# lxd99/TPNet

Hardware: AMD Instinct MI355X
Metric: temporal edges/sec (proj-update + pairwise readout) (higher is better)
Workload: dtype f32; 1 GPU; C2: Wikipedia-shape d=128 B=1000, L=3, synthetic S(8227,1000,E,span) stream of 2399000 edges, decoder-level unit (2 readouts + update per edge); batch=1000, dim=128, num_layer=3, nodes=9228, parallelism=single GPU

## Files before the change

### tpnet_amd/csrc/wplan_dense.hip

```cpp
#include "wplan_dense.hpp"

namespace tpnet {

static constexpr int64_t DENSE_SHARD_MAX_BATCH = 8192;
bool wplan_dense_eligible(int64_t N, int d, int L, int64_t batch) {
    static const int off = TPNET_DEV_INT(NO_PLAN_DENSE, 0);
    if (off || batch < 1 || batch > DENSE_SHARD_MAX_BATCH || N > (int64_t)DENSE_MAX_CHUNKS * 256) return false;
    return (int64_t)N * 12 <= batch * (int64_t)L * d * 4;
}

size_t wplan_dense_bytes(int64_t Ec, int64_t batch, int64_t N, int d, int L) {
    if (!wplan_dense_eligible(N, d, L, batch)) return 0;
    return measured([&](Arena& a) { DView v; dense_layout(a, v, Ec, batch, N); });
}

struct DArgs {
    const int64_t* src;
    const int64_t* dst;
    const int64_t* neg;
    const double* t;
    const double* t_prev;
    const NodeMeta* meta;
    uint32_t* err;
    int64_t Ec, Bfull, N, nb, nw;
    double now_time, lambda;
    int32_t node_bits, L, nwhich , nchunks;
    int64_t own;
    uint32_t* status;
};

__device__ __forceinline__ void dense_place(const WPlan& p, const WTmp& q, const DView& D, const DArgs& a,
                                            const uint32_t* __restrict__ lstart, const uint32_t* __restrict__ cbase,
                                            const double* tl, int64_t x) {
    const BatchDesc* __restrict__ desc = p.base.desc;
    const int KW = p.K;
    const int64_t b = x / (2 * a.Bfull);
    const int64_t e0b = b * a.Bfull;
    const int64_t neb = (a.Ec - e0b < a.Bfull) ? (a.Ec - e0b) : a.Bfull;
    const uint32_t node = q.bkey[x];
    const int32_t partner = q.bpart[x];
    const float coef = q.bcoef[x];
    const uint32_t ri = q.bri[x];
    const uint32_t fl = q.bflags[x] & WT_STRUCT_MASK;
    const uint32_t val = q.bval[x];
    const uint2 mo = D.m[b * D.Ns + node];
    const uint2 mp = D.m[b * D.Ns + (uint32_t)partner];
    const uint2 wsl_own = (fl & WREF_RUN_HEAD) ? D.wsl[(b / KW) * D.Ns + node] : make_uint2(0u, 0u);
    const uint32_t bo = D.base[node] + cbase[node / (uint32_t)DCH];
    const uint32_t bp = D.base[(uint32_t)partner] + cbase[(uint32_t)partner / (uint32_t)DCH];
    const uint4 o0 = reinterpret_cast<const uint4*>(a.meta + node)[0], o1 = reinterpret_cast<const uint4*>(a.meta + node)[1];
    const uint4 p0 = reinterpret_cast<const uint4*>(a.meta + partner)[0], p1 = reinterpret_cast<const uint4*>(a.meta + partner)[1];
    const double Tb = desc[b].t_last, Tnow = desc[b].now;
    const DVRef own = dense_version(desc, tl, mo, bo, o0, o1);
    const DVRef pr = dense_version(desc, tl, mp, bp, p0, p1);
    const uint32_t f = bo + mo.x + ri;
    uint32_t out = fl | pr.ref;
    float dec = 1.0f;
    if (fl & WREF_RUN_HEAD) {
        const int64_t w = b / KW;
        const uint32_t prevb = mo.y >> 16;
        const bool chain_head = mo.x == 0u || (int64_t)prevb < w * KW;
        if (chain_head) {
            float g_first = 1.0f;
            if (own.ref & WREF_TABLE) g_first = decay3_f32(a.lambda, Tb - own.t_src);
            else dec = decay3_f32(a.lambda, Tb - own.t_src);
            const uint32_t cnt = wsl_own.x;
            const int c = wchain_class(cnt, p.heavy_thr);
            const uint32_t pair = (uint32_t)w * 8u + (uint32_t)c;
            const uint32_t chunk = node / (uint32_t)DCH;
            const uint32_t at = lstart[pair] + D.cpre[(size_t)chunk * (size_t)(a.nw * 8) + pair] + D.crank[w * D.Ns + node];
            uint4* rec = reinterpret_cast<uint4*>(p.chains + at);
            rec[0] = make_uint4(f, cnt, node, own.ref);
            rec[1] = make_uint4(__float_as_uint(g_first), 0u, 0u, 0u);
        } else {
            dec = decay3_f32(a.lambda, Tb - own.t_src);
        }
    }
    if ((fl & WREF_RUN_TAIL) && D.lastb[node] == (uint32_t)b) out |= WREF_LAST_RUN;
    wrec_store(p.rec, f, partner, coef, out, decay3_f32(a.lambda, Tb - pr.t_src), dec, (int32_t)node, (uint32_t)b);
    if (a.nwhich >= 2) {
        const bool side = val >= (uint32_t)neb;
        const int64_t e = e0b + (side ? (int64_t)val - neb : (int64_t)val);
        p.e_ref[(side ? a.Ec : 0) + e] = own.ref;
        p.e_g[(side ? a.Ec : 0) + e] = decay3_f32(a.lambda, Tnow - own.t_src);
    }
}

__device__ __forceinline__ void dense_neg(const WPlan& p, const DView& D, const DArgs& a, const uint32_t* __restrict__ basef,
                                          int64_t e) {
    const BatchDesc* __restrict__ desc = p.base.desc;
    int64_t node = a.neg[e];
    if ((uint64_t)node >= (uint64_t)a.N) node = 0;
    const int64_t b = e / a.Bfull;
    const uint2 m = D.m[b * D.Ns + node];
    const uint32_t bs = basef[node];
    const uint4 m0 = reinterpret_cast<const uint4*>(a.meta + node)[0], m1 = reinterpret_cast<const uint4*>(a.meta + node)[1];
    const DVRef r = dense_version(desc, nullptr, m, bs, m0, m1);
    p.e_ref[2 * a.Ec + e] = r.ref;
    p.e_g[2 * a.Ec + e] = decay3_f32(a.lambda, desc[b].now - r.t_src);
}

__device__ __forceinline__ void dense_neg_c(const WPlan& p, const DView& D, const DArgs& a, const uint32_t* __restrict__ cbase,
                                            const double* tl, int64_t e, int which = 2) {
    const BatchDesc* __restrict__ desc = p.base.desc;
    int64_t node = which == 2 ? a.neg[e] : a.dst[e];
    if ((uint64_t)node >= (uint64_t)a.N) node = 0;
    if (which == 1 && node < a.own) return;
    const int64_t b = e / a.Bfull;
    const uint2 m = D.m[b * D.Ns + node];
    const uint32_t bs = D.base[node] + cbase[(uint32_t)node / (uint32_t)DCH];
    const uint4 m0 = reinterpret_cast<const uint4*>(a.meta + node)[0], m1 = reinterpret_cast<const uint4*>(a.meta + node)[1];
    const DVRef r = dense_version(desc, tl, m, bs, m0, m1);
    p.e_ref[(int64_t)which * a.Ec + e] = r.ref;
    p.e_g[(int64_t)which * a.Ec + e] = decay3_f32(a.lambda, desc[b].now - r.t_src);
}

template <int BS, int IPT>
__global__ __launch_bounds__(BS) void k_dense_sort(WPlan p, WTmp q, DView D, DArgs a) {
    __shared__ WSortShared<BS, IPT> sh;
    const int64_t bb = blockIdx.x;
    wsort_batch<BS, IPT, true>(sh, q, p.base.desc, a.src, a.dst, a.t, a.Ec, (int32_t)a.Bfull, a.N, a.node_bits, a.now_time,
                               a.t_prev, a.lambda, a.L, a.err, p.K, bb, D.len + bb * D.Ns);
}


static constexpr int DENSE_GROUP_MAX_N = 12288;
template <int BS, int IPT, int NT>
__global__ __launch_bounds__(BS) void k_dense_group(WPlan p, WTmp q, DView D, DArgs a) {
    constexpr int NC = BS * IPT;
    constexpr int SPT = NT / BS;
    static_assert(SPT * BS == NT && SPT % 4 == 0, "k_dense_group: table size");
    constexpr int NW = BS / 64;
    constexpr int BMW = NC / 32;
    constexpr uint32_t SMALL = 16;
    static_assert(NC <= 2048 && BMW <= 64, "k_dense_group: j fits 11 bits, a hub's bitmap one word per lane");
    const int64_t bb = blockIdx.x;
    const BatchSpan sp = batch_span(bb, a.src, a.dst, a.t, a.Ec, a.Bfull);
    const int64_t e0 = sp.e0;
    const int32_t B = sp.B;
    const int64_t g0 = 2 * e0;
    uint16_t* __restrict__ lenrow = D.len + bb * D.Ns;
    __shared__ __attribute__((aligned(16))) uint32_t tab[NT];
    __shared__ uint16_t mem[NC];
    __shared__ uint32_t sorted[NC];
    __shared__ uint32_t bm[NW][BMW];
    __shared__ uint32_t e_src[NC / 2], e_dst[NC / 2];
    __shared__ float e_w[NC / 2];
    __shared__ uint32_t n_big, wsum[NW];
    __shared__ uint32_t big[NC / SMALL];
    const int tid = threadIdx.x;
    const int nc = 2 * B;
    const auto burst = edges_load<BS, IPT / 2>(sp);
    const double t_now = batch_clock(bb, e0, a.t, a.t_prev, a.now_time);
    if (tid == 0) n_big = 0;
#pragma unroll
    for (int k = 0; k < SPT / 4; ++k) reinterpret_cast<uint4*>(tab)[k * BS + tid] = make_uint4(0u, 0u, 0u, 0u);
    edges_stage<BS>(burst, B, a.N, a.lambda, a.err, e_src, e_dst, e_w);
    __syncthreads();
    uint32_t key[IPT], arr[IPT];
#pragma unroll
    for (int k = 0; k < IPT; ++k) {
        const int j = k * BS + tid;
        key[k] = 0;
        arr[k] = 0;
        if (j < nc) {
            key[k] = contrib_target(j, B, e_src, e_dst);
            arr[k] = atomicAdd(&tab[key[k]], 1u);
        }
    }
    __syncthreads();
    uint32_t c[SPT], tsum = 0;
#pragma unroll
    for (int k = 0; k < SPT / 4; ++k) {
        const uint4 v = reinterpret_cast<const uint4*>(tab)[tid * (SPT / 4) + k];
        c[4 * k] = v.x; c[4 * k + 1] = v.y; c[4 * k + 2] = v.z; c[4 * k + 3] = v.w;
        tsum += v.x + v.y + v.z + v.w;
    }
#pragma unroll
    for (int k = 0; k < SPT; ++k) {
        const int64_t n = (int64_t)tid * SPT + k;
        if (n < a.N) lenrow[n] = (uint16_t)c[k];
    }
    uint32_t total;
    uint32_t base = block_excl_scan<BS, false>(tsum, wsum, total);
    if (tsum) {
#pragma unroll
        for (int k = 0; k < SPT; ++k) {
            tab[tid * SPT + k] = (base << 16) | c[k];
            if (c[k] > SMALL) big[atomicAdd(&n_big, 1u)] = (uint32_t)(tid * SPT + k);
            base += c[k];
        }
    }
    __syncthreads();
#pragma unroll
    for (int k = 0; k < IPT; ++k) {
        const int j = k * BS + tid;
        if (j < nc) mem[(tab[key[k]] >> 16) + arr[k]] = (uint16_t)j;
    }
    __syncthreads();
    rank_groups<BS, IPT, SMALL>(tab, key, nc, mem, big, n_big, bm, [&](uint32_t j, uint32_t gb, uint32_t rank, uint32_t cnt) {
        sorted[gb + rank] = j | (rank << 11) | ((cnt - 1u) << 22);
    });
    __syncthreads();
#pragma unroll
    for (int k = 0; k < IPT; ++k) {
        const int pos = k * BS + tid;
        if (pos < nc) {
            const uint32_t v = sorted[pos];
            const uint32_t j = v & 0x7FFu, ri = (v >> 11) & 0x7FFu, cnt = (v >> 22) + 1u;
            int32_t partner;
            float w;
            contrib_partner_weight((int)j, B, e_src, e_dst, e_w, partner, w);
            q.bkey[g0 + pos] = contrib_target((int)j, B, e_src, e_dst);
            q.bpart[g0 + pos] = partner;
            q.bcoef[g0 + pos] = w;
            q.bval[g0 + pos] = j;
            q.binv[g0 + j] = (uint32_t)(g0 + pos);
            q.bri[g0 + pos] = ri;
            q.bflags[g0 + pos] = wref_run_flags(ri, ri + 1u == cnt);
        }
    }
    if (tid == 0) batch_desc_store(p.base.desc, bb, sp, t_now, burst.t_last, 0u, 0u, false, a.lambda, a.L);
}

template <int BS, int IPT>
__global__ __launch_bounds__(BS) void k_dense_sort_shard(WPlan p, WTmp q, DView D, DArgs a) {
    using Sort = rocprim::block_radix_sort<uint32_t, BS, IPT, uint32_t>;
    constexpr int NC = BS * IPT;
    constexpr int CMAX = 16;
    __shared__ union U {
        typename Sort::storage_type sort;
        struct { uint32_t key[NC]; uint32_t ustart[NC]; } s;
        struct { uint32_t ckey[NC]; uint32_t cval[NC]; } c;
    } u;
    __shared__ uint32_t wsum[BS / 64];
    constexpr int HBITS = 2048;
    __shared__ uint32_t hbits[HBITS];
    static_assert(sizeof(U) + sizeof(uint32_t) * HBITS <= 62 * 1024, "k_dense_sort_shard: LDS budget");
    const int64_t bb = blockIdx.x;
    const int tid = threadIdx.x;
    const BatchSpan sp = batch_span(bb, a.src, a.dst, a.t, a.Ec, a.Bfull);
    const int64_t e0 = sp.e0;
    const int32_t B = sp.B;
    const int64_t* __restrict__ src = sp.src;
    const int64_t* __restrict__ dst = sp.dst;
    const double* __restrict__ t = sp.t;
    const int64_t g0 = 2 * e0;
    uint16_t* __restrict__ lenrow = D.len + bb * D.Ns;
    for (int i = tid; i < HBITS; i += BS) hbits[i] = 0u;
    const bool hfit = a.N - a.own <= (int64_t)HBITS * 32;
    for (int64_t n = tid; n < (hfit ? a.own : a.N); n += BS) lenrow[n] = 0;
    __syncthreads();
    const double t_last = t[B - 1];
    const int nall = 2 * B;
    const int C = (nall + BS - 1) / BS;
    uint32_t rk[CMAX];
    uint32_t kept = 0;
#pragma unroll
    for (int k = 0; k < CMAX; ++k) {
        rk[k] = 0xFFFFFFFFu;
        const int j = tid * C + k;
        if (k < C && j < nall) {
            const bool side = j >= B;
            const int e = side ? j - B : j;
            const int64_t sv = src[e], dv = dst[e];
            const bool ok = (uint64_t)sv < (uint64_t)a.N && (uint64_t)dv < (uint64_t)a.N;
            if (!ok) {
                if (!side) atomicAdd(a.err, 1u);
            } else {
                const int64_t tg = side ? dv : sv;
                if (tg < a.own) { rk[k] = (uint32_t)tg; ++kept; }
                else if (hfit) atomicOr(&hbits[(tg - a.own) >> 5], 1u << ((tg - a.own) & 31));
                else lenrow[tg] = 1;
            }
        }
    }
    uint32_t total;
    uint32_t off = block_excl_scan<BS>(kept, wsum, total);
    if (hfit)
        for (int64_t n = a.own + tid; n < a.N; n += BS) lenrow[n] = (uint16_t)((hbits[(n - a.own) >> 5] >> ((n - a.own) & 31)) & 1u);
    if (total > (uint32_t)NC) {
        if (tid == 0 && a.status) atomicAdd(a.status, 1u);
        total = NC;
    }
#pragma unroll
    for (int k = 0; k < CMAX; ++k) {
        if (rk[k] != 0xFFFFFFFFu) {
            if (off < (uint32_t)NC) { u.c.ckey[off] = rk[k]; u.c.cval[off] = (uint32_t)(tid * C + k); }
            ++off;
        }
    }
    __syncthreads();
    const int nc = (int)total;
    uint32_t keys[IPT], vals[IPT];
    const uint32_t pad_key = 1u << a.node_bits;
#pragma unroll
    for (int k = 0; k < IPT; ++k) {
        const int j = tid * IPT + k;
        keys[k] = j < nc ? u.c.ckey[j] : pad_key;
        vals[k] = j < nc ? u.c.cval[j] : 0u;
    }
    __syncthreads();
    Sort().sort(keys, vals, u.sort, 0u, (unsigned)(a.node_bits + 1));
    __syncthreads();
#pragma unroll
    for (int k = 0; k < IPT; ++k) u.s.key[tid * IPT + k] = keys[k];
    __syncthreads();
    uint32_t hcount = 0;
    bool hd[IPT];
#pragma unroll
    for (int k = 0; k < IPT; ++k) {
        const int j = tid * IPT + k;
        hd[k] = j < nc && (j == 0 || u.s.key[j - 1] != keys[k]);
        hcount += hd[k] ? 1u : 0u;
        if (j < nc) {
            const uint32_t val = vals[k];
            const bool side = val >= (uint32_t)B;
            const int e = side ? (int)val - B : (int)val;
            const int64_t sv = src[e], dv = dst[e];
            const float x = (float)t_last - (float)t[e];
            q.bkey[g0 + j] = keys[k];
            q.bpart[g0 + j] = (int32_t)(side ? sv : dv);
            q.bcoef[g0 + j] = expf((float)(-a.lambda) * x);
            q.bval[g0 + j] = val;
            q.binv[g0 + val] = (uint32_t)(g0 + j);
        }
    }
    uint32_t htotal;
    const uint32_t rank = block_excl_scan<BS>(hcount, wsum, htotal);
    uint32_t myrun[IPT];
    run_starts(hd, rank, u.s.ustart, myrun);
    __syncthreads();
    run_ranks_store(myrun, u.s.ustart, htotal, nc, q.bri + g0, q.bflags + g0);
    run_lengths_store<BS>(u.s.key, u.s.ustart, htotal, nc, lenrow);
    if (tid == 0)
        batch_desc_store(p.base.desc, bb, sp, batch_clock(bb, e0, a.t, a.t_prev, a.now_time), t_last, (uint32_t)nc, 0u, false,
                         a.lambda, a.L);
}

__global__ __launch_bounds__(DCH) void k_dense_win(WPlan p, DView D, DArgs a) {
    __shared__ uint32_t wcnt[(DCH / 64) * 8];
    const int tid = threadIdx.x, lane = tid & 63, wave = tid >> 6;
    const int KW = p.K;
    const int64_t c = blockIdx.x / a.nw, w = blockIdx.x - c * a.nw;
    const int64_t n = c * DCH + tid;
    const bool live = n < a.N;
    const int64_t nld = live ? n : 0;
    const int64_t bw0 = w * KW, bw1 = (bw0 + KW < a.nb) ? bw0 + KW : a.nb;
    uint32_t sum = 0, last = 0xFFFFu;
    constexpr int UB = 16;
    for (int64_t b0 = bw0; b0 < bw1; b0 += UB) {
        uint32_t l[UB];
#pragma unroll
        for (int k = 0; k < UB; ++k) {
            const int64_t b = (b0 + k < bw1) ? b0 + k : bw1 - 1;
            l[k] = (uint32_t)D.len[b * D.Ns + nld];
        }
#pragma unroll
        for (int k = 0; k < UB; ++k) {
            if (b0 + k < bw1) {
                sum += l[k];
                last = l[k] ? (uint32_t)(b0 + k) : last;
            }
        }
    }
    if (!live) sum = 0;
    if (live) D.wsl[w * D.Ns + n] = make_uint2(sum, last);
    const int cl = (sum && n < a.own) ? wchain_class(sum, p.heavy_thr) : -1;
    uint32_t myrank = 0;
#pragma unroll
    for (int c8 = 0; c8 < 8; ++c8) {
        const unsigned long long mk = __ballot(cl == c8);
        if (cl == c8) myrank = (uint32_t)__popcll(mk & ((1ull << lane) - 1ull));
        if (lane == 0) wcnt[wave * 8 + c8] = (uint32_t)__popcll(mk);
    }
    __syncthreads();
    if (cl >= 0) {
        for (int wv = 0; wv < wave; ++wv) myrank += wcnt[wv * 8 + cl];
        D.crank[w * D.Ns + n] = myrank;
    }
    if (tid < 8) {
        uint32_t tsum = 0;
        for (int wv = 0; wv < DCH / 64; ++wv) tsum += wcnt[wv * 8 + tid];
        D.ccnt[(size_t)c * (size_t)(a.nw * 8) + w * 8 + tid] = tsum;
    }
}

__global__ __launch_bounds__(DCH) void k_dense_pre(WPlan p, DView D, DArgs a) {
    __shared__ uint32_t wsum[DCH / 64];
    __shared__ uint32_t part[DCH];
    const int tid = threadIdx.x;
    const int KW = p.K;
    const int64_t c = blockIdx.x / a.nw, w = blockIdx.x - c * a.nw;
    const int64_t n = c * DCH + tid;
    const bool live = n < a.N;
    const int64_t nld = live ? n : 0;
    const int64_t bw0 = w * KW, bw1 = (bw0 + KW < a.nb) ? bw0 + KW : a.nb;
    const size_t npair = (size_t)(a.nw * 8);
    constexpr int UB = 16;
    {
        uint32_t ps = 0;
        for (int64_t cq = tid >> 3; cq < c; cq += DCH / 8) ps += D.ccnt[(size_t)cq * npair + w * 8 + (tid & 7)];
        part[tid] = ps;
    }
    uint32_t run = 0, prevb = 0xFFFFu;
    for (int64_t w0 = 0; w0 < w; w0 += UB) {
        uint2 v[UB];
#pragma unroll
        for (int k = 0; k < UB; ++k) {
            const int64_t wq = (w0 + k < w) ? w0 + k : w - 1;
            v[k] = D.wsl[wq * D.Ns + nld];
        }
#pragma unroll
        for (int k = 0; k < UB; ++k) {
            if (w0 + k < w) {
                run += v[k].x;
                prevb = v[k].x ? v[k].y : prevb;
            }
        }
    }
    for (int64_t b0 = bw0; b0 < bw1; b0 += UB) {
        uint32_t l[UB];
#pragma unroll
        for (int k = 0; k < UB; ++k) {
            const int64_t b = (b0 + k < bw1) ? b0 + k : bw1 - 1;
            l[k] = (uint32_t)D.len[b * D.Ns + nld];
        }
#pragma unroll
        for (int k = 0; k < UB; ++k) {
            const int64_t b = b0 + k;
            if (b < bw1) {
                if (live) D.m[b * D.Ns + n] = make_uint2(run, l[k] | (prevb << 16));
                run += l[k];
                prevb = l[k] ? (uint32_t)b : prevb;
            }
        }
    }
    __syncthreads();
    if (tid < 8) {
        uint32_t before = 0;
        for (int k = 0; k < DCH / 8; ++k) before += part[k * 8 + tid];
        D.cpre[(size_t)c * npair + w * 8 + tid] = before;
        if (c == a.nchunks - 1) D.ptot[w * 8 + tid] = before + D.ccnt[(size_t)c * npair + w * 8 + tid];
    }
    if (w == a.nw - 1) {
        if (!live) run = 0;
        uint32_t total;
        const uint32_t ex = block_excl_scan<DCH>(run, wsum, total);
        if (live) { D.tot[n] = run; D.lastb[n] = prevb; D.base[n] = ex; }
        if (tid == 0) D.ctot[c] = total;
    }
}

__global__ __launch_bounds__(DCH) void k_dense_place(WPlan p, WTmp q, DView D, DArgs a) {
    __shared__ uint32_t wsum[DCH / 64];
    __shared__ uint32_t cbase[DENSE_MAX_CHUNKS];
    __shared__ uint32_t lstart[DENSE_MAX_WINDOWS * 8];
    __shared__ double tlast[DENSE_TL];
    const int tid = threadIdx.x;
    const int npair = (int)a.nw * 8;
    const double* tl = a.nb <= DENSE_TL ? tlast : nullptr;
    if (tl)
        for (int64_t b = tid; b < a.nb; b += DCH) tlast[b] = p.base.desc[b].t_last;
    {
        uint32_t carry = 0;
        for (int64_t c0 = 0; c0 < a.nchunks; c0 += DCH) {
            const int64_t c = c0 + tid;
            const uint32_t v = c < a.nchunks ? D.ctot[c] : 0u;
            uint32_t tot;
            const uint32_t ex = block_excl_scan<DCH>(v, wsum, tot);
            if (c < a.nchunks) cbase[c] = carry + ex;
            carry += tot;
        }
        carry = 0;
        for (int i0 = 0; i0 < npair; i0 += DCH) {
            const int i = i0 + tid;
            const uint32_t v = i < npair ? D.ptot[i] : 0u;
            uint32_t tot;
            const uint32_t ex = block_excl_scan<DCH>(v, wsum, tot);
            if (i < npair) lstart[i] = carry + ex;
            carry += tot;
        }
        __syncthreads();
    }
    if (blockIdx.x == 0) {
        for (int64_t w = tid; w < a.nw; w += DCH) {
            uint32_t t8[8], n = 0;
#pragma unroll
            for (int k = 0; k < 8; ++k) { t8[k] = D.ptot[w * 8 + k]; n += t8[k]; }
            WinDesc W;
            W.start = lstart[w * 8];
            W.n_heavy = t8[0];
            W.n_chains = n;
            W.n_ext = t8[0] + t8[1] + t8[2];
            W.n_ext1 = t8[0] + t8[1];
            W.n_med = 0;
            for (int k = 0; k <= wchain_med_classes(p.heavy_thr); ++k) W.n_med += t8[k];
            W.pad1 = W.pad2 = 0;
            p.wdesc[w] = W;
        }
    }
    const int64_t gid = (int64_t)blockIdx.x * DCH + tid, gsz = (int64_t)gridDim.x * DCH;
    for (int64_t n = gid; n < a.N; n += gsz) D.basef[n] = D.base[n] + cbase[n / DCH];
    const int64_t nc = 2 * a.Ec;
    const bool shard = a.own < a.N;
    const int64_t n_neg = a.nwhich == 3 ? a.Ec : 0;
    const int64_t items = nc + n_neg + ((shard && a.nwhich >= 2) ? a.Ec : 0);
    for (int64_t x = gid; x < items; x += gsz) {
        if (x < nc) {
            if (shard) {
                const int64_t b = x / (2 * a.Bfull);
                if (x - 2 * b * a.Bfull >= (int64_t)p.base.desc[b].n_light) continue;
            }
            dense_place(p, q, D, a, lstart, cbase, tl, x);
        } else if (x < nc + n_neg) {
            dense_neg_c(p, D, a, cbase, tl, x - nc);
        } else {
            dense_neg_c(p, D, a, cbase, tl, x - nc - n_neg, 1);
        }
    }
}

__global__ __launch_bounds__(256) void k_wplan_dense_negs(WPlan p, DView D, DArgs a) {
    for (int64_t e = (int64_t)blockIdx.x * blockDim.x + threadIdx.x; e < a.Ec; e += (int64_t)gridDim.x * blockDim.x)
        dense_neg(p, D, a, D.basef, e);
}

__global__ __launch_bounds__(256) void k_wwriteback_dense(tpnet_state S, WPlan p, DView D, uint32_t bid, int64_t own) {
    constexpr int LANES = 32;
    const int per = S.L * S.d;
    const int pv = per / 4;
    NodeMeta* meta = reinterpret_cast<NodeMeta*>(S.meta);
    const int gl = threadIdx.x % LANES, g = threadIdx.x / LANES;
    constexpr int GPB = 256 / LANES;
    for (int64_t n = (int64_t)blockIdx.x * GPB + g; n < own; n += (int64_t)gridDim.x * GPB) {
        const uint32_t tot = D.tot[n];
        const uint32_t bs = D.basef[n], lb = D.lastb[n];
        const uint32_t ver = meta[n].ver;
        if (!tot) continue;
        const uint32_t pos = bs + tot - 1u;
        const int c = (int)(ver & 1u);
        const float4* __restrict__ srow = reinterpret_cast<const float4*>(p.log + (int64_t)pos * per);
        float4* __restrict__ drow = reinterpret_cast<float4*>(S.q + ((int64_t)(c ^ 1) * S.N + n) * (int64_t)per);
        for (int x = gl; x < pv; x += LANES) drow[x] = srow[x];
        if (gl == 0) publish_meta(meta + n, c ^ 1, p.base.desc[lb].t_last, bid);
    }
}

bool wplan_dense_applies(const tpnet_state& st, const WPlan& p, int64_t Ec, int64_t batch, int K) {
    return batch <= PLAN_ONE_MAX && wplan_dense_applies_shard(st, p, Ec, batch, K);
}
bool wplan_dense_applies_shard(const tpnet_state& st, const WPlan& p, int64_t Ec, int64_t batch, int K) {
    if (!p.dense || K < 1 || !wplan_dense_eligible(st.N, st.d, st.L, batch)) return false;
    const int64_t nb = (Ec + batch - 1) / batch;
    const int64_t nw = (nb + K - 1) / K;
    int node_bits = 1;
    while (node_bits < 63 && (1ll << node_bits) < st.N) ++node_bits;
    return nw <= DENSE_MAX_WINDOWS && nw <= (nb + 1) / 2 + 1 && nb < 65535 && node_bits <= 31 && 2 * Ec < (int64_t)WREF_SLOT_MASK;
}

int wplan_dense_build(const tpnet_state& st, const WPlan& p, const WPlanArgs& pa, hipStream_t s) {
    const int64_t Ec = pa.Ec, batch = pa.batch;
    const bool replay = pa.replay;
    const int64_t own = (pa.own < 0 || pa.own > st.N) ? st.N : pa.own;
    const bool shard = own < st.N;
    if (!(shard ? wplan_dense_applies_shard(st, p, Ec, batch, p.K) : wplan_dense_applies(st, p, Ec, batch, p.K))) return TPNET_ERR_BAD_ARG;
    if (shard && replay) return TPNET_ERR_BAD_ARG;
    const int64_t nb = (Ec + batch - 1) / batch;
    const WTmp q = wtmp_of(p, (size_t)(2 * Ec));
    const DView D = dview_of(p, Ec, batch, st.N);
    DArgs a;
    a.src = pa.src; a.dst = pa.dst; a.neg = pa.neg; a.t = pa.t; a.t_prev = pa.t_prev_dev;
    a.meta = reinterpret_cast<const NodeMeta*>(st.meta);
    a.err = st.err;
    a.Ec = Ec; a.Bfull = batch; a.N = st.N; a.nb = nb; a.nw = (nb + p.K - 1) / p.K;
    a.now_time = pa.now_time; a.lambda = pa.lambda;
    int node_bits = 1;
    while (node_bits < 31 && (1ll << node_bits) < st.N) ++node_bits;
    a.node_bits = node_bits;
    a.L = st.L;
    a.nwhich = pa.want_readout ? (pa.neg ? 3 : 2) : 0;
    a.nchunks = (int32_t)((st.N + DCH - 1) / DCH);
    a.own = own;
    a.status = pa.status;
    if (replay) {
        if (a.nwhich == 3) {
            hipLaunchKernelGGL(k_wplan_dense_negs, dim3(grid_1d(Ec, 2048)), dim3(256), 0, s, p, D, a);
            TPNET_HIP_TRY(hipGetLastError());
        }
        return TPNET_OK;
    }
#define TPNET_WDENSE(BS_, IPT_) hipLaunchKernelGGL((k_dense_sort<BS_, IPT_>), dim3((unsigned)nb), dim3(BS_), 0, s, p, q, D, a)
    const int64_t n2 = 2 * batch;
    static const int no_group = TPNET_DEV_INT(DENSE_SORT, 0);
    if (shard) hipLaunchKernelGGL((k_dense_sort_shard<1024, 4>), dim3((unsigned)nb), dim3(1024), 0, s, p, q, D, a);
    else if (!no_group && n2 <= 2048 && st.N <= DENSE_GROUP_MAX_N)
        hipLaunchKernelGGL((k_dense_group<1024, 2, DENSE_GROUP_MAX_N>), dim3((unsigned)nb), dim3(1024), 0, s, p, q, D, a);
    else TPNET_FOR_BATCH_TILE(n2, TPNET_WDENSE);
#undef TPNET_WDENSE
    const unsigned bgrid = (unsigned)((int64_t)a.nchunks * a.nw);
    hipLaunchKernelGGL(k_dense_win, dim3(bgrid), dim3(DCH), 0, s, p, D, a);
    hipLaunchKernelGGL(k_dense_pre, dim3(bgrid), dim3(DCH), 0, s, p, D, a);
    static_assert(DCH == 256, "grid_1d counts workgroups of 256");
    hipLaunchKernelGGL(k_dense_place, dim3(grid_1d(3 * Ec, 4096)), dim3(DCH), 0, s, p, q, D, a);
    TPNET_HIP_TRY(hipGetLastError());
    return TPNET_OK;
}

int wplan_dense_writeback(const tpnet_state& st, const WPlan& p, int64_t Ec, int64_t batch, uint32_t launch_id, hipStream_t s,
                          int64_t own) {
    if ((st.L * st.d) % 4 != 0) return TPNET_ERR_BAD_ARG;
    if (own < 0 || own > st.N) own = st.N;
    const DView D = dview_of(p, Ec, batch, st.N);
    int64_t grid = (own + 7) / 8;
    if (grid > 16384) grid = 16384;
    if (grid < 1) grid = 1;
    hipLaunchKernelGGL(k_wwriteback_dense, dim3((unsigned)grid), dim3(256), 0, s, st, p, D, launch_id, own);
    TPNET_HIP_TRY(hipGetLastError());
    return TPNET_OK;
}

}
```

Measured before the change: 367.1 million edges/s.

## Fuse dense window/prefix kernels and prefetch place items ahead of scans

Result: no change. 364.3 million edges/s (-0.7%).

```diff
diff --git a/tpnet_amd/csrc/wplan_dense.hip b/tpnet_amd/csrc/wplan_dense.hip
--- a/tpnet_amd/csrc/wplan_dense.hip
+++ b/tpnet_amd/csrc/wplan_dense.hip
@@ -29,60 +29,151 @@
     uint32_t* status;
 };
 
-__device__ __forceinline__ void dense_place(const WPlan& p, const WTmp& q, const DView& D, const DArgs& a,
-                                            const uint32_t* __restrict__ lstart, const uint32_t* __restrict__ cbase,
-                                            const double* tl, int64_t x) {
+struct DItem {
+    int32_t kind;
+    int64_t b, e;
+    uint32_t node;
+    int32_t partner;
+    float coef;
+    uint32_t ri, fl, val, n_light;
+    double Tb, Tnow;
+    uint2 mo, mp, wsl;
+    uint32_t bo, bp, crank, lastb;
+    uint4 o0, o1, p0, p1;
+};
+
+__device__ __forceinline__ void dense_item_load(DItem& it, const WPlan& p, const WTmp& q, const DArgs& a, int64_t nc, int64_t n_neg,
+                                                bool shard, int64_t x) {
     const BatchDesc* __restrict__ desc = p.base.desc;
-    const int KW = p.K;
-    const int64_t b = x / (2 * a.Bfull);
-    const int64_t e0b = b * a.Bfull;
-    const int64_t neb = (a.Ec - e0b < a.Bfull) ? (a.Ec - e0b) : a.Bfull;
-    const uint32_t node = q.bkey[x];
-    const int32_t partner = q.bpart[x];
-    const float coef = q.bcoef[x];
-    const uint32_t ri = q.bri[x];
-    const uint32_t fl = q.bflags[x] & WT_STRUCT_MASK;
-    const uint32_t val = q.bval[x];
-    const uint2 mo = D.m[b * D.Ns + node];
-    const uint2 mp = D.m[b * D.Ns + (uint32_t)partner];
-    const uint2 wsl_own = (fl & WREF_RUN_HEAD) ? D.wsl[(b / KW) * D.Ns + node] : make_uint2(0u, 0u);
-    const uint32_t bo = D.base[node] + cbase[node / (uint32_t)DCH];
-    const uint32_t bp = D.base[(uint32_t)partner] + cbase[(uint32_t)partner / (uint32_t)DCH];
-    const uint4 o0 = reinterpret_cast<const uint4*>(a.meta + node)[0], o1 = reinterpret_cast<const uint4*>(a.meta + node)[1];
-    const uint4 p0 = reinterpret_cast<const uint4*>(a.meta + partner)[0], p1 = reinterpret_cast<const uint4*>(a.meta + partner)[1];
-    const double Tb = desc[b].t_last, Tnow = desc[b].now;
-    const DVRef own = dense_version(desc, tl, mo, bo, o0, o1);
-    const DVRef pr = dense_version(desc, tl, mp, bp, p0, p1);
-    const uint32_t f = bo + mo.x + ri;
-    uint32_t out = fl | pr.ref;
-    float dec = 1.0f;
-    if (fl & WREF_RUN_HEAD) {
-        const int64_t w = b / KW;
-        const uint32_t prevb = mo.y >> 16;
-        const bool chain_head = mo.x == 0u || (int64_t)prevb < w * KW;
-        if (chain_head) {
-            float g_first = 1.0f;
-            if (own.ref & WREF_TABLE) g_first = decay3_f32(a.lambda, Tb - own.t_src);
-            else dec = decay3_f32(a.lambda, Tb - own.t_src);
-            const uint32_t cnt = wsl_own.x;
-            const int c = wchain_class(cnt, p.heavy_thr);
-            const uint32_t pair = (uint32_t)w * 8u + (uint32_t)c;
-            const uint32_t chunk = node / (uint32_t)DCH;
-            const uint32_t at = lstart[pair] + D.cpre[(size_t)chunk * (size_t)(a.nw * 8) + pair] + D.crank[w * D.Ns + node];
-            uint4* rec = reinterpret_cast<uint4*>(p.chains + at);
-            rec[0] = make_uint4(f, cnt, node, own.ref);
-            rec[1] = make_uint4(__float_as_uint(g_first), 0u, 0u, 0u);
-        } else {
-            dec = decay3_f32(a.lambda, Tb - own.t_src);
-        }
-    }
-    if ((fl & WREF_RUN_TAIL) && D.lastb[node] == (uint32_t)b) out |= WREF_LAST_RUN;
-    wrec_store(p.rec, f, partner, coef, out, decay3_f32(a.lambda, Tb - pr.t_src), dec, (int32_t)node, (uint32_t)b);
-    if (a.nwhich >= 2) {
-        const bool side = val >= (uint32_t)neb;
-        const int64_t e = e0b + (side ? (int64_t)val - neb : (int64_t)val);
-        p.e_ref[(side ? a.Ec : 0) + e] = own.ref;
-        p.e_g[(side ? a.Ec : 0) + e] = decay3_f32(a.lambda, Tnow - own.t_src);
+    it.kind = -1;
+    if (x < 0) return;
+    if (x < nc) {
+        it.kind = 0;
+        it.e = x;
+        it.b = x / (2 * a.Bfull);
+        it.node = q.bkey[x];
+        it.partner = q.bpart[x];
+        it.coef = q.bcoef[x];
+        it.ri = q.bri[x];
+        it.fl = q.bflags[x] & WT_STRUCT_MASK;
+        it.val = q.bval[x];
+        it.Tb = desc[it.b].t_last;
+        it.Tnow = desc[it.b].now;
+        it.n_light = shard ? desc[it.b].n_light : 0xFFFFFFFFu;
+    } else {
+        it.kind = x < nc + n_neg ? 2 : 1;
+        it.e = x - nc - (it.kind == 1 ? n_neg : 0);
+        it.b = it.e / a.Bfull;
+        const int64_t node = it.kind == 2 ? a.neg[it.e] : a.dst[it.e];
+        it.Tnow = desc[it.b].now;
+        it.partner = (uint64_t)node >= (uint64_t)a.N ? 0 : (int32_t)node;
+        if (it.kind == 1 && (int64_t)it.partner < a.own) it.kind = -1;
+    }
+}
+
+template <bool SHORT>
+__device__ __forceinline__ void dense_item_gather(DItem& it, const WPlan& p, const DView& D, const DArgs& a) {
+    if constexpr (SHORT) {
+        if (it.kind == 0 && it.e - 2 * it.b * a.Bfull >= (int64_t)it.n_light) it.kind = -1;
+        const uint32_t node = it.kind < 0 ? 0u : (it.kind == 0 ? it.node : (uint32_t)it.partner);
+        const uint32_t partner = it.kind == 0 ? (uint32_t)it.partner : node;
+        const int64_t b = it.kind < 0 ? 0 : it.b;
+        const int64_t w = b / p.K;
+        it.mo = D.m[b * D.Ns + node];
+        it.mp = D.m[b * D.Ns + partner];
+        it.wsl = D.wsl[w * D.Ns + node];
+        it.crank = D.crank[w * D.Ns + node];
+        it.lastb = D.lastb[node];
+        it.bo = D.base[node];
+        it.bp = D.base[partner];
+        it.o0 = reinterpret_cast<const uint4*>(a.meta + node)[0];
+        it.o1 = reinterpret_cast<const uint4*>(a.meta + node)[1];
+        it.p0 = reinterpret_cast<const uint4*>(a.meta + partner)[0];
+        it.p1 = reinterpret_cast<const uint4*>(a.meta + partner)[1];
+        return;
+    }
+    if (it.kind == 0) {
+        if (it.e - 2 * it.b * a.Bfull >= (int64_t)it.n_light) { it.kind = -1; return; }
+        const uint32_t node = it.node, partner = (uint32_t)it.partner;
+        const int64_t w = it.b / p.K;
+        const bool head = it.fl & WREF_RUN_HEAD;
+        it.mo = D.m[it.b * D.Ns + node];
+        it.mp = D.m[it.b * D.Ns + partner];
+        it.wsl = head ? D.wsl[w * D.Ns + node] : make_uint2(0u, 0u);
+        it.crank = 0u;
+        it.lastb = (it.fl & WREF_RUN_TAIL) ? D.lastb[node] : 0xFFFFFFFFu;
+        it.bo = D.base[node];
+        it.bp = D.base[partner];
+        it.o0 = reinterpret_cast<const uint4*>(a.meta + node)[0];
+        it.o1 = reinterpret_cast<const uint4*>(a.meta + node)[1];
+        it.p0 = reinterpret_cast<const uint4*>(a.meta + partner)[0];
+        it.p1 = reinterpret_cast<const uint4*>(a.meta + partner)[1];
+    } else if (it.kind > 0) {
+        const uint32_t node = (uint32_t)it.partner;
+        it.mo = D.m[it.b * D.Ns + node];
+        it.bo = D.base[node];
+        it.o0 = reinterpret_cast<const uint4*>(a.meta + node)[0];
+        it.o1 = reinterpret_cast<const uint4*>(a.meta + node)[1];
+    }
+}
+
+__device__ __forceinline__ void dense_item_finish(const DItem& it, const WPlan& p, const DView& D, const DArgs& a,
+                                                  const uint32_t* __restrict__ lstart, const uint32_t* __restrict__ cbase,
+                                                  const uint32_t* __restrict__ ctab, const double* tl) {
+    const BatchDesc* __restrict__ desc = p.base.desc;
+    if (it.kind == 0) {
+        const int KW = p.K;
+        const int64_t b = it.b;
+        const int64_t e0b = b * a.Bfull;
+        const int64_t neb = (a.Ec - e0b < a.Bfull) ? (a.Ec - e0b) : a.Bfull;
+        const uint32_t node = it.node, fl = it.fl;
+        const int32_t partner = it.partner;
+        const uint2 mo = it.mo;
+        const uint32_t bo = it.bo + cbase[node / (uint32_t)DCH];
+        const uint32_t bp = it.bp + cbase[(uint32_t)partner / (uint32_t)DCH];
+        const double Tb = it.Tb, Tnow = it.Tnow;
+        const DVRef own = dense_version(desc, tl, mo, bo, it.o0, it.o1);
+        const DVRef pr = dense_version(desc, tl, it.mp, bp, it.p0, it.p1);
+        const uint32_t f = bo + mo.x + it.ri;
+        uint32_t out = fl | pr.ref;
+        float dec = 1.0f;
+        if (fl & WREF_RUN_HEAD) {
+            const int64_t w = b / KW;
+            const uint32_t prevb = mo.y >> 16;
+            const bool chain_head = mo.x == 0u || (int64_t)prevb < w * KW;
+            if (chain_head) {
+                float g_first = 1.0f;
+                if (own.ref & WREF_TABLE) g_first = decay3_f32(a.lambda, Tb - own.t_src);
+                else dec = decay3_f32(a.lambda, Tb - own.t_src);
+                const uint32_t cnt = it.wsl.x;
+                const int c = wchain_class(cnt, p.heavy_thr);
+                const uint32_t pair = (uint32_t)w * 8u + (uint32_t)c;
+                const uint32_t chunk = node / (uint32_t)DCH;
+                const uint32_t before = ctab ? ctab[pair * (uint32_t)a.nchunks + chunk]
+                                             : D.cpre[(size_t)chunk * (size_t)(a.nw * 8) + pair];
+                const uint32_t rank = ctab ? it.crank : D.crank[w * D.Ns + node];
+                const uint32_t at = lstart[pair] + before + rank;
+                uint4* rec = reinterpret_cast<uint4*>(p.chains + at);
+                rec[0] = make_uint4(f, cnt, node, own.ref);
+                rec[1] = make_uint4(__float_as_uint(g_first), 0u, 0u, 0u);
+            } else {
+                dec = decay3_f32(a.lambda, Tb - own.t_src);
+            }
+        }
+        if ((fl & WREF_RUN_TAIL) && it.lastb == (uint32_t)b) out |= WREF_LAST_RUN;
+        wrec_store(p.rec, f, partner, it.coef, out, decay3_f32(a.lambda, Tb - pr.t_src), dec, (int32_t)node, (uint32_t)b);
+        if (a.nwhich >= 2) {
+            const bool side = it.val >= (uint32_t)neb;
+            const int64_t e = e0b + (side ? (int64_t)it.val - neb : (int64_t)it.val);
+            p.e_ref[(side ? a.Ec : 0) + e] = own.ref;
+            p.e_g[(side ? a.Ec : 0) + e] = decay3_f32(a.lambda, Tnow - own.t_src);
+        }
+    } else if (it.kind > 0) {
+        const uint32_t node = (uint32_t)it.partner;
+        const uint32_t bs = it.bo + cbase[node / (uint32_t)DCH];
+        const DVRef r = dense_version(desc, tl, it.mo, bs, it.o0, it.o1);
+        p.e_ref[(int64_t)it.kind * a.Ec + it.e] = r.ref;
+        p.e_g[(int64_t)it.kind * a.Ec + it.e] = decay3_f32(a.lambda, it.Tnow - r.t_src);
     }
 }
 
@@ -98,21 +189,6 @@
     const DVRef r = dense_version(desc, nullptr, m, bs, m0, m1);
     p.e_ref[2 * a.Ec + e] = r.ref;
     p.e_g[2 * a.Ec + e] = decay3_f32(a.lambda, desc[b].now - r.t_src);
-}
-
-__device__ __forceinline__ void dense_neg_c(const WPlan& p, const DView& D, const DArgs& a, const uint32_t* __restrict__ cbase,
-                                            const double* tl, int64_t e, int which = 2) {
-    const BatchDesc* __restrict__ desc = p.base.desc;
-    int64_t node = which == 2 ? a.neg[e] : a.dst[e];
-    if ((uint64_t)node >= (uint64_t)a.N) node = 0;
-    if (which == 1 && node < a.own) return;
-    const int64_t b = e / a.Bfull;
-    const uint2 m = D.m[b * D.Ns + node];
-    const uint32_t bs = D.base[node] + cbase[(uint32_t)node / (uint32_t)DCH];
-    const uint4 m0 = reinterpret_cast<const uint4*>(a.meta + node)[0], m1 = reinterpret_cast<const uint4*>(a.meta + node)[1];
-    const DVRef r = dense_version(desc, tl, m, bs, m0, m1);
-    p.e_ref[(int64_t)which * a.Ec + e] = r.ref;
-    p.e_g[(int64_t)which * a.Ec + e] = decay3_f32(a.lambda, desc[b].now - r.t_src);
 }
 
 template <int BS, int IPT>
@@ -452,21 +528,155 @@
     }
 }
 
+static constexpr int DENSE_SHORT_NB = 32;
+static constexpr int DENSE_SHORT_NW = DENSE_SHORT_NB / 2 + 1;
+static constexpr int DENSE_SHORT_TAB = 4096;
+static inline bool dense_short_plan(int64_t nb, int64_t nchunks, int64_t nw) {
+    return nb <= DENSE_SHORT_NB && nw <= DENSE_SHORT_NW && nchunks * nw * 8 <= DENSE_SHORT_TAB;
+}
+__global__ __launch_bounds__(DCH) void k_dense_winpre(WPlan p, DView D, DArgs a) {
+    __shared__ uint32_t wcnt[(DCH / 64) * 8];
+    __shared__ uint32_t wsum[DCH / 64];
+    const int tid = threadIdx.x, lane = tid & 63, wave = tid >> 6;
+    const int KW = p.K;
+    const int64_t c = blockIdx.x / a.nw, w = blockIdx.x - c * a.nw;
+    const int64_t n = c * DCH + tid;
+    const bool live = n < a.N;
+    const int64_t nld = live ? n : 0;
+    const int bw0 = (int)(w * KW), bw1 = (int)((w * KW + KW < a.nb) ? w * KW + KW : a.nb);
+    uint32_t l[DENSE_SHORT_NB];
+#pragma unroll
+    for (int k = 0; k < DENSE_SHORT_NB; ++k) {
+        const int b = k < bw1 ? k : bw1 - 1;
+        l[k] = (uint32_t)D.len[(int64_t)b * D.Ns + nld];
+    }
+    uint32_t run = 0, prevb = 0xFFFFu;
+    uint32_t sum = 0, last = 0xFFFFu;
+#pragma unroll
+    for (int k = 0; k < DENSE_SHORT_NB; ++k) {
+        if (k < bw1) {
+            if (k >= bw0) {
+                if (live) D.m[(int64_t)k * D.Ns + n] = make_uint2(run, l[k] | (prevb << 16));
+                sum += l[k];
+                last = l[k] ? (uint32_t)k : last;
+            }
+            run += l[k];
+            prevb = l[k] ? (uint32_t)k : prevb;
+        }
+    }
+    if (!live) sum = 0;
+    if (live) D.wsl[w * D.Ns + n] = make_uint2(sum, last);
+    const int cl = (sum && n < a.own) ? wchain_class(sum, p.heavy_thr) : -1;
+    uint32_t myrank = 0;
+#pragma unroll
+    for (int c8 = 0; c8 < 8; ++c8) {
+        const unsigned long long mk = __ballot(cl == c8);
+        if (cl == c8) myrank = (uint32_t)__popcll(mk & ((1ull << lane) - 1ull));
+        if (lane == 0) wcnt[wave * 8 + c8] = (uint32_t)__popcll(mk);
+    }
+    __syncthreads();
+    if (cl >= 0) {
+        for (int wv = 0; wv < wave; ++wv) myrank += wcnt[wv * 8 + cl];
+        D.crank[w * D.Ns + n] = myrank;
+    }
+    if (tid < 8) {
+        uint32_t tsum = 0;
+        for (int wv = 0; wv < DCH / 64; ++wv) tsum += wcnt[wv * 8 + tid];
+        D.ccnt[(size_t)c * (size_t)(a.nw * 8) + w * 8 + tid] = tsum;
+    }
+    if (w == a.nw - 1) {
+        if (!live) run = 0;
+        uint32_t total;
+        const uint32_t ex = block_excl_scan<DCH, false>(run, wsum, total);
+        if (live) { D.tot[n] = run; D.lastb[n] = prevb; D.base[n] = ex; }
+        if (tid == 0) D.ctot[c] = total;
+    }
+}
+
+__device__ __forceinline__ uint32_t wave_incl_scan_dpp(uint32_t v) {
+    int x = (int)v;
+    x += __builtin_amdgcn_update_dpp(0, x, 0x111 , 0xF, 0xF, false);
+    x += __builtin_amdgcn_update_dpp(0, x, 0x112 , 0xF, 0xF, false);
+    x += __builtin_amdgcn_update_dpp(0, x, 0x114 , 0xF, 0xF, false);
+    x += __builtin_amdgcn_update_dpp(0, x, 0x118 , 0xF, 0xF, false);
+    x += __builtin_amdgcn_update_dpp(0, x, 0x142 , 0xA, 0xF, false);
+    x += __builtin_amdgcn_update_dpp(0, x, 0x143 , 0xC, 0xF, false);
+    return (uint32_t)x;
+}
+
+template <bool SHORT>
 __global__ __launch_bounds__(DCH) void k_dense_place(WPlan p, WTmp q, DView D, DArgs a) {
     __shared__ uint32_t wsum[DCH / 64];
     __shared__ uint32_t cbase[DENSE_MAX_CHUNKS];
     __shared__ uint32_t lstart[DENSE_MAX_WINDOWS * 8];
     __shared__ double tlast[DENSE_TL];
+    __shared__ uint32_t ctab[SHORT ? DENSE_SHORT_TAB : 1];
+    __shared__ uint32_t ptl[SHORT ? DENSE_SHORT_NW * 8 : 1];
     const int tid = threadIdx.x;
     const int npair = (int)a.nw * 8;
     const double* tl = a.nb <= DENSE_TL ? tlast : nullptr;
-    if (tl)
-        for (int64_t b = tid; b < a.nb; b += DCH) tlast[b] = p.base.desc[b].t_last;
+    const int64_t gid = (int64_t)blockIdx.x * DCH + tid, gsz = (int64_t)gridDim.x * DCH;
+    const int64_t nc = 2 * a.Ec;
+    const bool shard = a.own < a.N;
+    const int64_t n_neg = a.nwhich == 3 ? a.Ec : 0;
+    const int64_t items = nc + n_neg + ((shard && a.nwhich >= 2) ? a.Ec : 0);
+    DItem it;
+    if constexpr (SHORT) dense_item_load(it, p, q, a, nc, n_neg, shard, gid < items ? gid : -1);
+    const uint32_t ct0 = tid < a.nchunks ? D.ctot[tid] : 0u;
+    const double tl0 = p.base.desc[tid < a.nb ? tid : 0].t_last;
+    uint32_t pt0 = 0;
+    constexpr int CW = 4, CPASS = CW * (DCH / 64);
+    const int lane = tid & 63, wave = tid >> 6;
+    auto ccnt_load = [&](int col0, int c0, uint32_t (&v)[CW]) {
+#pragma unroll
+        for (int k = 0; k < CW; ++k) {
+            const int col = col0 + wave * CW + k, ch = c0 + lane;
+            const bool in = col < npair && ch < a.nchunks;
+            const uint32_t x = D.ccnt[in ? ch * npair + col : 0];
+            v[k] = in ? x : 0u;
+        }
+    };
+    uint32_t cv0[CW];
+    if constexpr (SHORT) ccnt_load(0, 0, cv0);
+    else pt0 = tid < npair ? D.ptot[tid] : 0u;
+    if constexpr (SHORT) dense_item_gather<SHORT>(it, p, D, a);
+    if (tl) {
+        if (tid < a.nb) tlast[tid] = tl0;
+        for (int64_t b = tid + DCH; b < a.nb; b += DCH) tlast[b] = p.base.desc[b].t_last;
+    }
+    if constexpr (SHORT) {
+        for (int col0 = 0; col0 < npair; col0 += CPASS) {
+            uint32_t before[CW];
+#pragma unroll
+            for (int k = 0; k < CW; ++k) before[k] = 0;
+            for (int c0 = 0; c0 < a.nchunks; c0 += 64) {
+                uint32_t v[CW];
+                if (col0 == 0 && c0 == 0) {
+#pragma unroll
+                    for (int k = 0; k < CW; ++k) v[k] = cv0[k];
+                } else {
+                    ccnt_load(col0, c0, v);
+                }
+#pragma unroll
+                for (int k = 0; k < CW; ++k) {
+                    const int col = col0 + wave * CW + k, ch = c0 + lane;
+                    const uint32_t inc = wave_incl_scan_dpp(v[k]);
+                    if (col < npair && ch < a.nchunks) ctab[col * a.nchunks + ch] = before[k] + inc - v[k];
+                    before[k] += (uint32_t)__builtin_amdgcn_readlane((int)inc, 63);
+                }
+            }
+#pragma unroll
+            for (int k = 0; k < CW; ++k) {
+                const int col = col0 + wave * CW + k;
+                if (lane == 0 && col < npair) ptl[col] = before[k];
+            }
+        }
+    }
     {
         uint32_t carry = 0;
         for (int64_t c0 = 0; c0 < a.nchunks; c0 += DCH) {
             const int64_t c = c0 + tid;
-            const uint32_t v = c < a.nchunks ? D.ctot[c] : 0u;
+            const uint32_t v = c0 == 0 ? ct0 : (c < a.nchunks ? D.ctot[c] : 0u);
             uint32_t tot;
             const uint32_t ex = block_excl_scan<DCH>(v, wsum, tot);
             if (c < a.nchunks) cbase[c] = carry + ex;
@@ -475,7 +685,9 @@
         carry = 0;
         for (int i0 = 0; i0 < npair; i0 += DCH) {
             const int i = i0 + tid;
-            const uint32_t v = i < npair ? D.ptot[i] : 0u;
+            uint32_t v;
+            if constexpr (SHORT) v = i < npair ? ptl[i] : 0u;
+            else v = i0 == 0 ? pt0 : (i < npair ? D.ptot[i] : 0u);
             uint32_t tot;
             const uint32_t ex = block_excl_scan<DCH>(v, wsum, tot);
             if (i < npair) lstart[i] = carry + ex;
@@ -487,7 +699,7 @@
         for (int64_t w = tid; w < a.nw; w += DCH) {
             uint32_t t8[8], n = 0;
 #pragma unroll
-            for (int k = 0; k < 8; ++k) { t8[k] = D.ptot[w * 8 + k]; n += t8[k]; }
+            for (int k = 0; k < 8; ++k) { t8[k] = SHORT ? ptl[w * 8 + k] : D.ptot[w * 8 + k]; n += t8[k]; }
             WinDesc W;
             W.start = lstart[w * 8];
             W.n_heavy = t8[0];
@@ -500,25 +712,15 @@
             p.wdesc[w] = W;
         }
     }
-    const int64_t gid = (int64_t)blockIdx.x * DCH + tid, gsz = (int64_t)gridDim.x * DCH;
+    const uint32_t* cpre_lds = SHORT ? ctab : nullptr;
+    for (int64_t x = gid; x < items; x += gsz) {
+        if (!SHORT || x != gid) {
+            dense_item_load(it, p, q, a, nc, n_neg, shard, x);
+            dense_item_gather<SHORT>(it, p, D, a);
+        }
+        dense_item_finish(it, p, D, a, lstart, cbase, cpre_lds, tl);
+    }
     for (int64_t n = gid; n < a.N; n += gsz) D.basef[n] = D.base[n] + cbase[n / DCH];
-    const int64_t nc = 2 * a.Ec;
-    const bool shard = a.own < a.N;
-    const int64_t n_neg = a.nwhich == 3 ? a.Ec : 0;
-    const int64_t items = nc + n_neg + ((shard && a.nwhich >= 2) ? a.Ec : 0);
-    for (int64_t x = gid; x < items; x += gsz) {
-        if (x < nc) {
-            if (shard) {
-                const int64_t b = x / (2 * a.Bfull);
-                if (x - 2 * b * a.Bfull >= (int64_t)p.base.desc[b].n_light) continue;
-            }
-            dense_place(p, q, D, a, lstart, cbase, tl, x);
-        } else if (x < nc + n_neg) {
-            dense_neg_c(p, D, a, cbase, tl, x - nc);
-        } else {
-            dense_neg_c(p, D, a, cbase, tl, x - nc - n_neg, 1);
-        }
-    }
 }
 
 __global__ __launch_bounds__(256) void k_wplan_dense_negs(WPlan p, DView D, DArgs a) {
@@ -599,10 +801,16 @@
     else TPNET_FOR_BATCH_TILE(n2, TPNET_WDENSE);
 #undef TPNET_WDENSE
     const unsigned bgrid = (unsigned)((int64_t)a.nchunks * a.nw);
-    hipLaunchKernelGGL(k_dense_win, dim3(bgrid), dim3(DCH), 0, s, p, D, a);
-    hipLaunchKernelGGL(k_dense_pre, dim3(bgrid), dim3(DCH), 0, s, p, D, a);
     static_assert(DCH == 256, "grid_1d counts workgroups of 256");
-    hipLaunchKernelGGL(k_dense_place, dim3(grid_1d(3 * Ec, 4096)), dim3(DCH), 0, s, p, q, D, a);
+    const dim3 cgrid(grid_1d(3 * Ec, 4096));
+    if (dense_short_plan(nb, a.nchunks, a.nw)) {
+        hipLaunchKernelGGL(k_dense_winpre, dim3(bgrid), dim3(DCH), 0, s, p, D, a);
+        hipLaunchKernelGGL(k_dense_place<true>, cgrid, dim3(DCH), 0, s, p, q, D, a);
+    } else {
+        hipLaunchKernelGGL(k_dense_win, dim3(bgrid), dim3(DCH), 0, s, p, D, a);
+        hipLaunchKernelGGL(k_dense_pre, dim3(bgrid), dim3(DCH), 0, s, p, D, a);
+        hipLaunchKernelGGL(k_dense_place<false>, cgrid, dim3(DCH), 0, s, p, q, D, a);
+    }
     TPNET_HIP_TRY(hipGetLastError());
     return TPNET_OK;
 }
```
